# uga-ssrl/SSRLCV

Measured on AMD Instinct MI355X. Metric: Mpix/s SIFT extract (+ Mmatches/s 128-D brute-force, see `matcher`), higher is better.
Workload: dtype f32; 1 GPU; 2-view 4096x4096 pair per GPU (tools/scene.py pinhole views (PCG32 terrain + texture through Image::Camera)): SIFT_FeatureFactory::generateFeatures (sparse DoG path) on each image, pixels resident in HBM; images_per_gpu=2, parallelism=image-pair shard, library=release build (libssrlcv_hip_release.so)

## Files before the change

### ssrlcv_amd/csrc/keypoints.hip

```cpp
#include <hip/hip_runtime.h>
#include <float.h>
#include <math.h>
#include <stdlib.h>
#include "compact.h"
#include "dev_switch.h"
#include "scan_lookback.h"
#include "device_math.h"
#include "sift_plan.h"
#include "ssrlcv_hip.h"

using svp::OctaveState;

namespace {

struct LevelSet {
  const float* lvl[svp::kGauss];
  const float* lvlMinMax;
  const float* minmax;
  const float2* polar;
  int w, h;
};

struct DogView {
  const float* lo;
// ... 473 lines not shown
  }
  tab->total = pos;
}
__device__ __forceinline__ int range_of(const RangeTable* tab, uint32_t u) {
  int r = 0;
#pragma unroll
  for (int k = 1; k < 20; ++k)
    if (tab->start[k] <= u) r = k;
  return r;
}

struct OctaveSet {
  LevelSet L[svp::kOctaves];
  const ssrlcv_sskeypoint* kps[svp::kOctaves];
  float pixelWidth[svp::kOctaves];
  float* thetas[svp::kOctaves];
  uint32_t* thetaCnt[svp::kOctaves];
  const void* consts[svp::kOctaves];
};

template <int MAXO, int LPKS>
__global__ __launch_bounds__(64) void k_thetas(const OctaveState* states, const RangeTable* tab, OctaveSet set, float lambda,
                                               float orientationThreshold) {
  constexpr int LANES = 1 << LPKS, PER_BLOCK = 64 >> LPKS, CW = kThetaChunk * LANES;
  __shared__ float s_hist[36][PER_BLOCK];
  if (blockIdx.x >= tab->total) return;
  const int range = __builtin_amdgcn_readfirstlane(range_of(tab, blockIdx.x));
  const int octave = range & 3, useg = kSegOrder[range >> 2];
  const LevelSet& L = set.L[octave];
  const float pixelWidth = set.pixelWidth[octave];
  const int t = threadIdx.x, sub = t & (LANES - 1), col = t >> LPKS;
  const float fsub2 = (float)(2 * sub);
  const uint32_t local = (blockIdx.x - tab->start[range]) * PER_BLOCK + (uint32_t)(t >> LPKS);
  const bool have = local < tab->count[range];
  const int gi = (int)(tab->first[range] + local);
  const float pi = SSRLCV_PI_F;
  const float rad10 = pi / 18.0f;
  const float inv10 = 1.0f / rad10;
  ssrlcv_sskeypoint kp;
  kp.loc.x = kp.loc.y = 0.0f;
  kp.sigma = 1.0f;
  if (have) kp = set.kps[octave][gi];
  const float kx = kp.loc.x, ky = kp.loc.y;
  const float windowWidth = ceilf(kp.sigma * 3.0f * lambda / pixelWidth);
  const float minx = kx - windowWidth, miny = ky - windowWidth, maxx = kx + windowWidth, maxy = ky + windowWidth;
  const bool inside = have && useg >= 1 && useg <= 3 &&
                      !(minx < 0.0f || miny < 0.0f || maxx >= (unsigned)(L.w - 1) || maxy >= (unsigned)(L.h - 1));
#pragma unroll
  for (int i = 0; i < 36 * PER_BLOCK / 64; ++i) (&s_hist[0][0])[i * 64 + t] = 0.0f;
  const float weight = 2.0f * lambda * lambda * kp.sigma * kp.sigma;
  const float rweight = 1.0f / weight;
  const int W = L.w;
  const size_t levelStride = svp::polar_level_stride(L.w, L.h);
  {
    const float2* base = L.polar + (size_t)(useg - 1) * levelStride;
    const __amdgpu_buffer_rsrc_t rsrc = __builtin_amdgcn_make_buffer_rsrc((void*)base, 0, (int)(uint32_t)(levelStride * 8), 0x00020000);
    typedef unsigned u32x4 __attribute__((ext_vector_type(4)));
    typedef unsigned u32x2 __attribute__((ext_vector_type(2)));
    struct Cursor { float x, y, ty2; unsigned rowoff; bool act; };
    Cursor cf;
    cf.x = minx;
    cf.y = miny;
    cf.ty2 = (miny - ky) * (miny - ky);
    cf.rowoff = (unsigned)round_pos(miny) * (unsigned)W + 1u;
    cf.act = inside;
    auto advance = [&](Cursor& c) {
      float xn = c.x + (float)CW;
      if (__any(c.act && !(c.x >= (float)CW))) {
        float ch = c.x;
#pragma unroll 8
        for (int i = 0; i < CW; ++i) ch += 1.0f;
        xn = c.x >= (float)CW ? xn : ch;
      }
      if (c.act) {
        if (xn <= maxx) {
          c.x = xn;
        } else {
          c.x = minx;
          c.y += 1.0f;
          if (!(c.y <= maxy)) c.act = false;
          const float ty = c.y - ky;
          c.ty2 = ty * ty;
          c.rowoff = (unsigned)round_pos(c.y) * (unsigned)W + 1u;
        }
      }
    };
    typedef u32x4 Chunk[kThetaChunk / 2];
    auto fetch = [&](const Cursor& c, Chunk& into) {
      if (!c.act) return;
      const unsigned off = (c.rowoff + (unsigned)round_pos(c.x)) * 8u + 16u * (unsigned)sub;
#pragma unroll
      for (int j = 0; j < kThetaChunk / 4; ++j) into[j] = __builtin_amdgcn_raw_buffer_load_b128(rsrc, (int)(off + 16u * LANES * j), 0, 0);
    };
    auto fetch_upper = [&](const Cursor& c, Chunk& into) {
      if (!c.act) return;
      const unsigned off = (c.rowoff + (unsigned)round_pos(c.x)) * 8u + 16u * (unsigned)sub;
#pragma unroll
      for (int j = kThetaChunk / 4; j < kThetaChunk / 2; ++j) into[j] = __builtin_amdgcn_raw_buffer_load_b128(rsrc, (int)(off + 16u * LANES * j), 0, 0);
    };
    auto wants_upper = [&](const Cursor& c) { return __any(c.act && c.x + (float)(CW / 2 - 1) <= maxx); };
    Chunk qa, qb;
    Cursor ca, cb;
#pragma unroll
    for (int j = 0; j < kThetaChunk / 2; ++j) qa[j] = qb[j] = u32x4{0u, 0u, 0u, 0u};
    ca = cf;
    fetch(cf, qa);
    if (wants_upper(cf)) fetch_upper(cf, qa);
    advance(cf);
    cb = cf;
    auto step = [&](Chunk& cur, const Cursor& cc, Chunk& nxt, Cursor& cn) __attribute__((always_inline)) {
      cn = cf;
      fetch(cf, nxt);
      if (wants_upper(cf)) fetch_upper(cf, nxt);
      advance(cf);
      float xs[kThetaChunk];
      float xlast = cc.x + (float)(CW - 1);
#pragma unroll
      for (int i = 0; i < kThetaChunk; ++i) xs[i] = cc.x + (fsub2 + (float)(((i >> 1) << (1 + LPKS)) | (i & 1)));
      if (__any(cc.act && !(cc.x >= (float)CW))) {
        float ch = cc.x;
        float xc[kThetaChunk];
#pragma unroll
        for (int sIdx = 0; sIdx < CW; ++sIdx) {
          const int q = (sIdx >> 1) & (LANES - 1), i = ((sIdx >> (1 + LPKS)) << 1) | (sIdx & 1);
          if (LANES == 1 || q == 0) xc[i] = ch;
          else xc[i] = sub == q ? ch : xc[i];
          if (sIdx + 1 < CW) ch += 1.0f;
        }
        const bool direct = cc.x >= (float)CW;
#pragma unroll
        for (int i = 0; i < kThetaChunk; ++i) xs[i] = direct ? xs[i] : xc[i];
        xlast = direct ? xlast : ch;
      }
      const float cty2 = cc.ty2;
      const unsigned crow = cc.rowoff;
      const bool cact = cc.act;
      const bool aligned = cc.x >= 4.0f && round_pos(xlast) == round_pos(cc.x) + (CW - 1);
      if (__any(cact && !aligned)) {
        if (cact && !aligned) {
#pragma unroll
          for (int i = 0; i < kThetaChunk; ++i) {
            u32x2 e = u32x2{0u, 0u};
            if (xs[i] <= maxx) e = __builtin_amdgcn_raw_buffer_load_b64(rsrc, (int)((crow + (unsigned)round_pos(xs[i])) * 8u), 0, 0);
            cur[i >> 1][(i & 1) * 2] = e[0];
            cur[i >> 1][(i & 1) * 2 + 1] = e[1];
          }
        }
      }
      auto weigh = [&](float ang, float xi, float& wgt, int& bin) {
        const float angle = fmod_2pi_above(ang + (2.0f * pi), 2.0f * pi);
        bin = (int)floorf(sv::exact_div3(angle, rad10, inv10));
        const float tx = xi - kx;
        wgt = sv::expf_nonpos(sv::exact_div5(-((tx * tx) + cty2), weight, rweight));
      };
      const bool upperHalf = __any(cact && xs[kThetaChunk / 2] <= maxx);
      float wg[kThetaChunk], mg[kThetaChunk];
      float* slot[kThetaChunk];
      auto weigh_half = [&](auto hc) __attribute__((always_inline)) {
        constexpr int i0 = decltype(hc)::value * (kThetaChunk / 2);
#pragma unroll
        for (int i = i0; i < i0 + kThetaChunk / 2; ++i) {
          const unsigned um = cur[i >> 1][(i & 1) * 2], ua = cur[i >> 1][(i & 1) * 2 + 1];
          int bin;
          weigh(__builtin_bit_cast(float, ua), xs[i], wg[i], bin);
          const bool counts = cact && xs[i] <= maxx && (unsigned)bin < 36u;
          slot[i] = &s_hist[counts ? bin : 0][col];
          mg[i] = counts ? __builtin_bit_cast(float, um) : 0.0f;
        }
      };
      auto vote_half = [&](auto hc) __attribute__((always_inline)) {
        constexpr int j0 = decltype(hc)::value * (kThetaChunk / 4);
#pragma unroll
        for (int j = j0; j < j0 + kThetaChunk / 4; ++j) {
#pragma unroll
          for (int q = 0; q < LANES; ++q) {
            if (LANES == 1 || sub == q) {
              const float h0 = *slot[2 * j], h1 = *slot[2 * j + 1];
              const float n0 = fmaf(mg[2 * j], wg[2 * j], h0);
              const float n1 = fmaf(mg[2 * j + 1], wg[2 * j + 1], slot[2 * j + 1] == slot[2 * j] ? n0 : h1);
              *slot[2 * j] = n0;
              *slot[2 * j + 1] = n1;
            }
            if (LANES > 1) __builtin_amdgcn_wave_barrier();
          }
        }
      };
      weigh_half(std::integral_constant<int, 0>{});
      if (upperHalf) weigh_half(std::integral_constant<int, 1>{});
      vote_half(std::integral_constant<int, 0>{});
      if (upperHalf) vote_half(std::integral_constant<int, 1>{});
    };
    while (__any(ca.act)) {
      step(qa, ca, qb, cb);
      if (!__any(cb.act)) break;
      step(qb, cb, qa, ca);
    }
  }
  uint32_t cnt = 0;
  float outTheta[MAXO];
#pragma unroll
  for (int i = 0; i < MAXO; ++i) outTheta[i] = -FLT_MAX;
  if (inside && sub == 0) {
    float maxHist = 0.0f;
    for (int i = 0; i < 36; ++i) {
      const float h = s_hist[i][col];
      if (h > maxHist) maxHist = h;
    }
    maxHist *= orientationThreshold;
    float bestMag[MAXO], bestTh[MAXO];
#pragma unroll
    for (int i = 0; i < MAXO; ++i) { bestMag[i] = 0.0f; bestTh[i] = 0.0f; }
    float hprev = s_hist[35][col], hb = s_hist[0][col];
    for (int b = 0; b < 36; ++b) {
      const float hnext = s_hist[b == 35 ? 0 : b + 1][col];
      if (!(hb < maxHist || hb < hprev || hb < hnext || hb < bestMag[MAXO - 1])) {
        float tmag = hb;
        float tt = (hprev - hnext) / (hprev - (2.0f * hb) + hnext);
        tt *= (pi / 36.0f);
        tt += (b * rad10);
        tt = fmodf(tt + (2.0f * pi), 2.0f * pi);
#pragma unroll
        for (int i = 0; i < MAXO; ++i) {
          if (tmag > bestMag[i]) {
#pragma unroll
            for (int ii = i; ii < MAXO; ++ii) {
              float m2 = bestMag[ii], t2 = bestTh[ii];
              bestMag[ii] = tmag;
              bestTh[ii] = tt;
              tmag = m2;
              tt = t2;
            }
          }
        }
      }
      hprev = hb;
      hb = hnext;
    }
#pragma unroll
    for (int i = 0; i < MAXO; ++i) {
      if (bestMag[i] != 0.0f) { outTheta[i] = bestTh[i]; cnt = i + 1; }
    }
  }
  if (have && sub == 0) {
#pragma unroll
    for (int i = 0; i < MAXO; ++i) set.thetas[octave][(size_t)gi * svp::kMaxOrient + i] = outTheta[i];
    set.thetaCnt[octave][gi] = cnt;
  }
}

__device__ __forceinline__ float uniform_f(float v) {
  return __builtin_bit_cast(float, __builtin_amdgcn_readfirstlane(__builtin_bit_cast(int, v)));
}
struct DescConst {
  float c, s;
  float windowWidth;
  float invExpDen;
  float voteScale;
  float invBin;
  uint32_t magic;
  int32_t segment;
};
static_assert(sizeof(DescConst) == 32, "one s_load_dwordx8");
__global__ __launch_bounds__(256) void k_desc_consts(const RangeTable* tab, OctaveSet set, float lambda, const OctaveState* states,
                                                     const GroupCtl* regularCtl) {
  const uint32_t total = tab->total;
  const bool fromTable = regularCtl != nullptr && regularCtl->regular != 0u;
  for (uint32_t u = blockIdx.x * 256 + threadIdx.x; u < total; u += gridDim.x * 256) {
    const int range = range_of(tab, u);
    const int octave = range & 3;
    const int i = (int)(tab->first[range] + (u - tab->start[range]));
    const ssrlcv_sskeypoint* kps = set.kps[octave];
    const float pixelWidth = set.pixelWidth[octave];
    DescConst* __restrict__ out = (DescConst*)const_cast<void*>(set.consts[octave]);
    DescConst d;
    const float theta = kps[i].theta;
    d.c = sv_cosf(-theta);
    d.s = sv_sinf(-theta);
    d.windowWidth = ceilf(kps[i].sigma * lambda / pixelWidth);
    d.invExpDen = 1.0f / (2.0f * d.windowWidth * d.windowWidth);
    int boundExp;
    (void)frexpf(1.4143f * ((d.windowWidth + 2.0f) * (d.windowWidth + 2.0f)), &boundExp);
    d.voteScale = ldexpf(1.0f, 31 - boundExp);
    d.invBin = 1.0f / (d.windowWidth / 2.0f);
    const unsigned wi = (unsigned)(int)d.windowWidth;
    d.magic = wi > 1u ? 0xFFFFFFFFu / wi + 1u : 0u;
    d.segment = fromTable ? kSegOrder[range >> 2] : segment_of(states + octave, i);
    out[i] = d;
  }
}

__device__ __forceinline__ unsigned vote_u32(float v) {
  int r;
  asm("v_cvt_rpi_i32_f32 %0, %1" : "=v"(r) : "v"(v));
  return (unsigned)r;
}

#ifndef SSRLCV_DESC_COPIES
#define SSRLCV_DESC_COPIES 8
#endif
constexpr int kDescCopies = SSRLCV_DESC_COPIES;
#ifndef SSRLCV_DESC_VGPRS
#define SSRLCV_DESC_VGPRS 64
#endif
__global__ __launch_bounds__(256) __attribute__((amdgpu_waves_per_eu(4, 8), amdgpu_num_vgpr(SSRLCV_DESC_VGPRS), amdgpu_num_sgpr(102))) void k_descriptors(const RangeTable* tab, OctaveSet set, const uint32_t* featBase,
                                                     ssrlcv_sift_feature* __restrict__ features, uint32_t maxFeatures) {
  __shared__ unsigned s_bins[4][(1 + 128 + 2) * kDescCopies];
  __shared__ __attribute__((aligned(8))) uint8_t s_bytes[4][128];
  const int lane = threadIdx.x & 63, wave = __builtin_amdgcn_readfirstlane(threadIdx.x >> 6);
  unsigned* bins = s_bins[wave] + kDescCopies;
  const int copy = lane & (kDescCopies - 1);
  const float pi = SSRLCV_PI_F;
  const float rad45 = pi / 4.0f;
  const float inv45 = 1.0f / rad45;
  const uint32_t totalUnits = tab->total;
  for (uint32_t unit = blockIdx.x * 4 + wave; unit < totalUnits; unit += gridDim.x * 4) {
    const int range = range_of(tab, unit);
    const int octave = range & 3;
    const int gi = (int)(tab->first[range] + (unit - tab->start[range]));
    const LevelSet& L = set.L[octave];
    const float pixelWidth = set.pixelWidth[octave];
    const float2* __restrict__ polar = L.polar;
    const DescConst dc = reinterpret_cast<const DescConst*>(set.consts[octave])[gi];
    const ssrlcv_sskeypoint kp = set.kps[octave][gi];
    const int seg = dc.segment;
    const float kx = kp.loc.x, ky = kp.loc.y;
    const float theta = kp.theta;
    const float windowWidth = dc.windowWidth;
    const float binWidth = windowWidth / 2.0f;
    const float c = dc.c, s = dc.s;
    const float2* __restrict__ pl = polar + (size_t)(seg - 1) * svp::polar_level_stride(L.w, L.h) + 1;
#pragma unroll
    for (int i = 0; i < 2 * kDescCopies; ++i) bins[i * 64 + lane] = 0u;
    f32x2 rc[16];
    {
      const int ci = lane & 15;
      const float hx = ((float)(ci >> 2) * 0.5f - 0.75f) * windowWidth, hy = ((float)(ci & 3) * 0.5f - 0.75f) * windowWidth;
      const float rx = (hx * c) + (hy * s), ry = (-hx * s) + (hy * c);
#pragma unroll
      for (int cell = 0; cell < 16; ++cell) {
        if ((cell >> 2) == 0 || (cell & 3) == 0) continue;
        rc[cell].x = __builtin_bit_cast(float, __builtin_amdgcn_readlane(__builtin_bit_cast(int, rx), cell));
        rc[cell].y = __builtin_bit_cast(float, __builtin_amdgcn_readlane(__builtin_bit_cast(int, ry), cell));
      }
    }
    const float expDen = 2.0f * windowWidth * windowWidth, invExpDen = dc.invExpDen, invBin = dc.invBin;
    const float voteScale = dc.voteScale;
    const int Wi = (int)windowWidth;
    const unsigned centreIdx = (unsigned)(Wi * (Wi + 1));
    const unsigned magic = dc.magic;
    auto sample = [&](unsigned idx, float& cx, float& cy, bool& ok) {
      const unsigned yq = Wi == 1 ? idx : __umulhi(idx, magic);
      const unsigned xq = idx - yq * (unsigned)Wi + 1u;
      const bool centre = idx >= centreIdx;
      const float x = centre ? 0.0f : (float)(int)xq;
      const float y = centre ? 0.0f : (float)(int)yq;
      cx = (x * c) + (y * s);
      cy = (-x * s) + (y * c);
      ok = idx <= centreIdx && fmaxf(fabsf(cx), fabsf(cy)) <= windowWidth;
    };
    auto gather = [&](float px, float py) { return polar_px(pl, L.w, round_coord(px), round_coord(py)); };
    auto split = [&](float2 pg, bool live, float& w0, float& w1, unsigned*& pa, float& ang, bool& odd) {
      ang = fmod_2pi_above(pg.y - theta + (2.0f * pi), 2.0f * pi);
      const float t45 = ang * inv45;
      const float fk = floorf(t45);
      const float u = t45 - fk;
      odd = live && !(u > 1.0e-4f && u < 0.9999f);
      int k0 = (int)fk;
      const float a0 = fabsf(ang - (fk * rad45)), a1 = fabsf(ang - ((fk + 1.0f) * rad45));
      w0 = (live && !odd && (unsigned)k0 < 8u) ? 1.0f - sv::exact_div3(a0, rad45, inv45) : 0.0f;
      w1 = (live && !odd && (unsigned)(k0 + 1) < 8u) ? 1.0f - sv::exact_div3(a1, rad45, inv45) : 0.0f;
      k0 = k0 < -1 ? -1 : k0;
      pa = bins + k0 * kDescCopies + copy;
    };
    float ncx, ncy;
    bool nok;
    sample((unsigned)lane, ncx, ncy, nok);
    float2 npg[4] = {make_float2(0.0f, 0.0f), make_float2(0.0f, 0.0f), make_float2(0.0f, 0.0f), make_float2(0.0f, 0.0f)};
    auto gather4 = [&]() {
      npg[0] = gather(ncx + kx, ncy + ky);
      npg[1] = gather(kx - ncy, ncx + ky);
      npg[2] = gather(kx - ncx, ky - ncy);
      npg[3] = gather(ncy + kx, ky - ncx);
    };
    if (nok) gather4();
    for (unsigned base = 0; base <= centreIdx; base += 64) {
      const float cx = ncx, cy = ncy;
      const bool ok = nok;
      const float2 pg0 = npg[0], pg1 = npg[1], pg2 = npg[2], pg3 = npg[3];
      const bool turned = ok && base + (unsigned)lane < centreIdx;
      sample(base + 64 + (unsigned)lane, ncx, ncy, nok);
      if (nok) gather4();
      const float r2n = -((cx * cx) + (cy * cy));
      const float g = sv::expf_nonpos(sv::exact_div3(r2n, expDen, invExpDen)) * voteScale;
      float a0, a1, b0, b1, c0, c1, d0, d1, angA, angB, angC, angD;
      bool oddA, oddB, oddC, oddD;
      unsigned *pa, *pb, *pc, *pd;
      split(pg0, ok, a0, a1, pa, angA, oddA);
      split(pg1, turned, b0, b1, pb, angB, oddB);
      split(pg2, turned, c0, c1, pc, angC, oddC);
      split(pg3, turned, d0, d1, pd, angD, oddD);
      const float magA = pg0.x * g, magB = pg1.x * g, magC = pg2.x * g, magD = pg3.x * g;
      const float bwl = ok ? binWidth : -1.0f;
#pragma unroll
      for (int cell = 0; cell < 16; ++cell) {
        const int nx = cell >> 2, ny = cell & 3;
        if (nx == 0 || ny == 0) continue;
        const int cellB = (3 - ny) * 4 + nx, cellC = 15 - cell, cellD = ny * 4 + (3 - nx);
        const float tx = fabsf(rc[cell].x - cx), ty = fabsf(rc[cell].y - cy);
        if (fmaxf(tx, ty) <= bwl) {
          const float wxy = (1.0f - sv::exact_div3(tx, binWidth, invBin)) * (1.0f - sv::exact_div3(ty, binWidth, invBin));
          atomicAdd(pa + cell * 8 * kDescCopies, vote_u32((wxy * a0) * magA));
          atomicAdd(pa + cell * 8 * kDescCopies + kDescCopies, vote_u32((wxy * a1) * magA));
          atomicAdd(pb + cellB * 8 * kDescCopies, vote_u32((wxy * b0) * magB));
          atomicAdd(pb + cellB * 8 * kDescCopies + kDescCopies, vote_u32((wxy * b1) * magB));
          atomicAdd(pc + cellC * 8 * kDescCopies, vote_u32((wxy * c0) * magC));
          atomicAdd(pc + cellC * 8 * kDescCopies + kDescCopies, vote_u32((wxy * c1) * magC));
          atomicAdd(pd + cellD * 8 * kDescCopies, vote_u32((wxy * d0) * magD));
          atomicAdd(pd + cellD * 8 * kDescCopies + kDescCopies, vote_u32((wxy * d1) * magD));
        }
      }
      if (__ballot(oddA || oddB || oddC || oddD) != 0ull) {
#pragma unroll 1
        for (int m = 0; m < 4; ++m) {
          const bool odd = m == 0 ? oddA : m == 1 ? oddB : m == 2 ? oddC : oddD;
          if (!odd) continue;
          const float mcx = m == 0 ? cx : m == 1 ? -cy : m == 2 ? -cx : cy;
          const float mcy = m == 0 ? cy : m == 1 ? cx : m == 2 ? -cy : -cx;
          const float mang = m == 0 ? angA : m == 1 ? angB : m == 2 ? angC : angD;
          const float mmag = m == 0 ? magA : m == 1 ? magB : m == 2 ? magC : magD;
#pragma unroll 1
          for (int cell = 0; cell < 16; ++cell) {
            const int ci = lane & 15;
            (void)ci;
            const float hx0 = ((float)(cell >> 2) * 0.5f - 0.75f) * windowWidth, hy0 = ((float)(cell & 3) * 0.5f - 0.75f) * windowWidth;
            const float rx = (hx0 * c) + (hy0 * s), ry = (-hx0 * s) + (hy0 * c);
            float hx = fabsf(rx - mcx), hy = fabsf(ry - mcy);
            if (hx <= binWidth && hy <= binWidth) {
              hx = hx / binWidth;
              hy = hy / binWidth;
              for (int k = 0; k < 8; ++k) {
                float angle = fabsf(mang - ((float)k * rad45));
                if (angle < rad45) {
                  angle /= rad45;
                  const float temp = (1.0f - hx) * (1.0f - hy) * (1.0f - angle) * mmag;
                  atomicAdd(bins + (cell * 8 + k) * kDescCopies + copy, vote_u32(temp));
                }
              }
            }
          }
        }
      }
    }
    __builtin_amdgcn_wave_barrier();
    unsigned t0 = 0u, t1 = 0u;
#pragma unroll
    for (int cpy = 0; cpy < kDescCopies; ++cpy) {
      t0 += bins[lane * kDescCopies + cpy];
      t1 += bins[(lane + 64) * kDescCopies + cpy];
    }
    float v0 = (float)t0, v1 = (float)t1;
    float sq = sqrtf(sv::wave_sum((v0 * v0) + (v1 * v1)));
    v0 = v0 / sq;
    v1 = v1 / sq;
    if (v0 > 0.2f) v0 = 0.2f;
    if (v1 > 0.2f) v1 = 0.2f;
    sq = sqrtf(sv::wave_sum((v0 * v0) + (v1 * v1)));
    {
      int b0 = lane, b1 = lane + 64;
      int o0 = (((b0 >> 3) & 3) * 4 + (b0 >> 5)) * 8 + (b0 & 7);
      int o1 = (((b1 >> 3) & 3) * 4 + (b1 >> 5)) * 8 + (b1 & 7);
      s_bytes[wave][o0] = (uint8_t)roundf(255.0f * v0 / sq);
      s_bytes[wave][o1] = (uint8_t)roundf(255.0f * v1 / sq);
    }
    __builtin_amdgcn_wave_barrier();
    const uint32_t fi = featBase[octave] + (uint32_t)gi;
    if (fi < maxFeatures) {
      ssrlcv_sift_feature* f = features + fi;
      if (lane < 16) *reinterpret_cast<uint2*>(&f->values[lane * 8]) = *reinterpret_cast<const uint2*>(&s_bytes[wave][lane * 8]);
      if (lane == 16) {
        f->parent = -1;
        f->theta = kp.theta;
        f->sigma = kp.sigma;
        f->loc.x = kp.loc.x * pixelWidth;
        f->loc.y = kp.loc.y * pixelWidth;
      }
    }
    __builtin_amdgcn_wave_barrier();
  }
}

LevelSet make_levels(const ssrlcv_sift_plan* plan, char* ws, int o) {
  LevelSet L;
  const svp::OctavePlan& oc = plan->oct[o];
  for (int b = 0; b < svp::kGauss; ++b) L.lvl[b] = (const float*)(ws + plan->off_gauss[o][b]);
  L.lvlMinMax = (const float*)(ws + plan->off_minmax) + (size_t)o * 2 * (svp::kGauss + svp::kDog);
  L.minmax = L.lvlMinMax + 2 * svp::kGauss;
  L.polar = (const float2*)(ws + oc.off_polar);
  L.w = (int)oc.w;
  L.h = (int)oc.h;
  return L;
}

void launch_polar(const ssrlcv_sift_plan* plan, char* ws, hipStream_t st, int oFirst = 0, int oLast = svp::kOctaves - 1) {
  PolarJobs jobs;
  uint32_t pos = 0;
  for (int o = 0; o < svp::kOctaves; ++o) {
    const svp::OctavePlan& oc = plan->oct[o];
    jobs.L[o] = make_levels(plan, ws, o);
    jobs.out[o] = (float2*)(ws + oc.off_polar);
    jobs.start[o] = pos;
    jobs.tilesX[o] = (oc.w + 255) / 256;
    if (o >= oFirst && o <= oLast) pos += jobs.tilesX[o] * ((oc.h + kPolRows - 1) / kPolRows);
  }
  jobs.start[svp::kOctaves] = pos;
  hipLaunchKernelGGL(k_polar, dim3(pos), dim3(256), 0, st, jobs);
}

}
namespace svp {
void launch_polar_octave(const ssrlcv_sift_plan* plan, char* ws, int octave, hipStream_t st) {
  PolarJobs jobs;
  const svp::OctavePlan& oc = plan->oct[octave];
  const uint32_t tilesX = (oc.w + 255) / 256, tiles = tilesX * ((oc.h + kPolRows - 1) / kPolRows);
  for (int o = 0; o < svp::kOctaves; ++o) {
    jobs.L[o] = make_levels(plan, ws, octave);
    jobs.out[o] = (float2*)(ws + oc.off_polar);
    jobs.tilesX[o] = tilesX;
    jobs.start[o] = o <= octave ? 0u : tiles;
  }
  jobs.start[svp::kOctaves] = tiles;
  hipLaunchKernelGGL(k_polar, dim3(tiles), dim3(256), 0, st, jobs);
}
}
namespace {
hipError_t run_discard(OctaveState* st, const ssrlcv_sskeypoint* src, ssrlcv_sskeypoint* dst, uint32_t cap,
                       uint32_t* words, hipStream_t stream) {
  const OctaveState* cst = st;
  auto keyfn = [=] __device__(uint32_t i) -> uint32_t {
    if (!cst->hasExtrema || (int)i >= cst->n) return 0u;
    if (src[i].discard) return 0u;
    return 1u << segment_of(cst, (int)i);
  };
  auto emit = [=] __device__(uint32_t i, int, uint32_t d) { dst[d] = src[i]; };
  uint32_t* totals = nullptr;
  auto post = [=] __device__(const uint32_t* tot) { book_discard(st, tot); };
  return svc::partition<svp::kDog, 8>(cap, keyfn, emit, words, &totals, stream, &st->n, 1u, post);
}

constexpr unsigned kWaveKernelOversubscription = 16;
inline unsigned list_blocks(uint32_t cap) {
  unsigned b = (cap + 255) / 256;
  return b > 1024 ? 1024 : b;
}

}

extern "C" {

int ssrlcv_sift_plan_keypoints(const ssrlcv_sift_plan* plan, void* workspace, int octave, ssrlcv_sskeypoint** list,
                               int** blurIndices_dev) {
  if (!plan || !workspace || octave < 0 || octave >= svp::kOctaves) return SSRLCV_ERR_INVALID_ARG;
  char* ws = (char*)workspace;
  if (list) *list = (ssrlcv_sskeypoint*)(ws + (plan->listInB[octave] ? plan->oct[octave].off_kpB : plan->oct[octave].off_kpA));
  if (blurIndices_dev) *blurIndices_dev = (int*)(ws + plan->off_state + sizeof(OctaveState) * octave);
  return SSRLCV_OK;
}

int ssrlcv_sift_plan_overflow(const ssrlcv_sift_plan* plan, const void* workspace, uint32_t* octaveMask,
                              ssrlcv_stream_t stream) {
  if (!plan || !workspace || !octaveMask) return SSRLCV_ERR_INVALID_ARG;
  OctaveState st[svp::kOctaves];
  SSRLCV_HIP_TRY(hipMemcpyAsync(st, (const char*)workspace + plan->off_state, sizeof st, hipMemcpyDeviceToHost,
                                (hipStream_t)stream));
  SSRLCV_HIP_TRY(hipStreamSynchronize((hipStream_t)stream));
  uint32_t m = 0;
  for (int o = 0; o < svp::kOctaves; ++o)
    if (st[o].overflow) m |= 1u << o;
  *octaveMask = m;
  return m ? SSRLCV_ERR_CAPACITY : SSRLCV_OK;
}

}
namespace {

struct ListCtx {
  const ssrlcv_sift_plan* plan;
  const svp::OctavePlan* oc;
  int o;
  hipStream_t s;
  OctaveState* st;
  LevelSet L;
  ssrlcv_sskeypoint *A, *B;
  uint8_t* flags;
  uint32_t* words;
  uint32_t cap;
  ssrlcv_sskeypoint* cur() const { return plan->listInB[o] ? B : A; }
  ssrlcv_sskeypoint* oth() const { return plan->listInB[o] ? A : B; }
  void flip() const { plan->listInB[o] ^= 1; }
};
ListCtx make_ctx(const ssrlcv_sift_plan* plan, char* ws, int o, hipStream_t s) {
  ListCtx c;
  c.plan = plan;
  c.oc = &plan->oct[o];
  c.o = o;
  c.s = s;
  c.st = (OctaveState*)(ws + plan->off_state) + o;
  c.L = make_levels(plan, ws, o);
  c.A = (ssrlcv_sskeypoint*)(ws + c.oc->off_kpA);
  c.B = (ssrlcv_sskeypoint*)(ws + c.oc->off_kpB);
  c.flags = (uint8_t*)(ws + c.oc->off_flags);
  c.words = (uint32_t*)(ws + c.oc->off_part);
  c.cap = c.oc->cap;
  return c;
}

int stage_extrema(const ListCtx& c, bool afterFirstNoise) {
  hipLaunchKernelGGL(k_state_reset, dim3(1), dim3(1), 0, c.s, c.st);
  c.plan->listInB[c.o] = 0;
  const uint32_t P = c.oc->w * c.oc->h, cap = c.cap;
  const int W = (int)c.oc->w;
  const int octaveId = c.o;
  const float s1 = c.oc->sigma[1], s2 = c.oc->sigma[2], s3 = c.oc->sigma[3];
  const LevelSet Lc = c.L;
  ssrlcv_sskeypoint* first = c.A;
  auto emit = [=] __device__(uint32_t p, int b, uint32_t d) {
    if (d >= cap) return;
    ssrlcv_sskeypoint kp;
    kp.octave = octaveId;
    kp.blur = (int)b + 1;
    kp.loc.x = (float)(p % W);
    kp.loc.y = (float)(p / W);
    kp.intensity = dog_view(Lc, b + 1).raw(p);
    kp.sigma = b == 0 ? s1 : b == 1 ? s2 : s3;
    kp.theta = -1.0f;
    kp.discard = 0;
    first[d] = kp;
  };
  uint32_t* totals = nullptr;
  hipError_t e = svc::partition_flags<3>(P, c.flags, afterFirstNoise ? svp::kNoiseFlagShift : 0, emit, c.words, &totals, c.s);
  if (e != hipSuccess) return (int)e;
  hipLaunchKernelGGL(k_book_extrema, dim3(1), dim3(1), 0, c.s, c.st, totals, cap);
  return SSRLCV_OK;
}
int discard_flagged(const ListCtx& c) {
  hipError_t e = run_discard(c.st, c.cur(), c.oth(), c.cap, c.words, c.s);
  if (e != hipSuccess) return (int)e;
  c.flip();
  return SSRLCV_OK;
}
int stage_noise(const ListCtx& c, float threshold) {
  hipLaunchKernelGGL(k_flag_noise, dim3(list_blocks(c.cap)), dim3(256), 0, c.s, c.st, c.cur(), threshold);
  return discard_flagged(c);
}
int stage_refine(const ListCtx& c) {
  hipLaunchKernelGGL(k_refine, dim3(list_blocks(c.cap)), dim3(256), 0, c.s, c.st, c.cur(), c.L, c.oc->sigma[0],
                     c.oc->sigma[1] / c.oc->sigma[0]);
  int rc = discard_flagged(c);
  if (rc) return rc;
  OctaveState* st = c.st;
  const OctaveState* cst = c.st;
  const ssrlcv_sskeypoint* src = c.cur();
  ssrlcv_sskeypoint* dst = c.oth();
  auto keyfn = [=] __device__(uint32_t i) -> uint32_t {
    if (!cst->hasExtrema || (int)i >= cst->n) return 0u;
    int b = src[i].blur;
    return (b < 0 || b >= svp::kDog) ? 0u : (1u << b);
  };
  auto emit = [=] __device__(uint32_t i, int, uint32_t d) { dst[d] = src[i]; };
  uint32_t* totals = nullptr;
  auto post = [=] __device__(const uint32_t* tot) { book_rescan(st, tot); };
  hipError_t e = svc::partition<svp::kDog, 8>(c.cap, keyfn, emit, c.words, &totals, c.s, &st->n, 1u, post);
  if (e != hipSuccess) return (int)e;
  c.flip();
  return SSRLCV_OK;
}
int stage_edges(const ListCtx& c) {
  hipLaunchKernelGGL(k_flag_edges, dim3(list_blocks(c.cap)), dim3(256), 0, c.s, c.st, c.cur(), c.L, svp::kEdgeThreshold);
  return discard_flagged(c);
}
int stage_window(const ListCtx& c) {
  hipLaunchKernelGGL(k_flag_window, dim3(list_blocks(c.cap)), dim3(256), 0, c.s, c.st, c.cur(), c.L.w, c.L.h, c.oc->pixelWidth,
                     c.plan->params.descriptorContribWidth);
  return discard_flagged(c);
}
int stage_noise_edges_window(const ListCtx& c) {
  hipLaunchKernelGGL(k_flag_noise_edges_window, dim3(list_blocks(c.cap)), dim3(256), 0, c.s, c.st, c.cur(), c.L, svp::kNoiseThreshold,
                     svp::kEdgeThreshold, c.oc->pixelWidth, c.plan->params.descriptorContribWidth);
  return discard_flagged(c);
}

OctaveSet make_set(const ssrlcv_sift_plan* plan, char* ws) {
  OctaveSet set;
  for (int o = 0; o < svp::kOctaves; ++o) {
    const svp::OctavePlan& oc = plan->oct[o];
    set.L[o] = make_levels(plan, ws, o);
    set.kps[o] = (const ssrlcv_sskeypoint*)(ws + (plan->listInB[o] ? oc.off_kpB : oc.off_kpA));
    set.pixelWidth[o] = oc.pixelWidth;
    set.thetas[o] = (float*)(ws + oc.off_theta);
    set.thetaCnt[o] = (uint32_t*)(ws + oc.off_thetaCnt);
    set.consts[o] = ws + oc.off_descConst;
  }
  return set;
}

constexpr int kExpandItems = 16;
__global__ __launch_bounds__(svs::kThreads) void k_expand_orient(OctaveState* st, const ssrlcv_sskeypoint* __restrict__ src,
                                                                 ssrlcv_sskeypoint* __restrict__ dst, const float* __restrict__ thetas,
                                                                 const uint32_t* __restrict__ thetaCnt, uint32_t maxO, uint32_t cap,
                                                                 svs::TileScan<1> ts, GroupCtl* ctl, int g, int pieces) {
  constexpr int ITEMS = kExpandItems;
  constexpr uint32_t kTile = svs::kThreads * ITEMS;
  const uint32_t n = st->hasExtrema && st->n > 0 ? (uint32_t)st->n : 0u;
  uint32_t lo = 0, hi = n;
  if (pieces > 1) {
    if (g > 0) lo = ctl->cut[g - 1] < n ? ctl->cut[g - 1] : n;
    if (g + 1 < pieces) hi = ctl->cut[g] < n ? ctl->cut[g] : n;
    if (hi < lo) hi = lo;
  }
  const uint32_t e0 = lo * maxO, e1 = hi * maxO;
  const uint32_t tiles = (e1 - e0 + kTile - 1) / kTile;
  const uint32_t before = ctl->totals[g];
  uint32_t segFirst[svp::kDog];
// ... 856 lines not shown
```

Measured before the change: 3585 Mpix/s.

## Compact descriptor cell voting via LDS cell table and bitmask loop, halve VGPR cap

The unrolled 9-cell vote loop, which issued eight LDS atomics per cell under divergent branches, becomes two steps. First a bitmask of the cells that pass is built, then a ctz-driven loop reads each cell's rotated centre and precomputed byte offsets from a small per-wave LDS table. The VGPR limit for k_descriptors is halved to allow more waves per SIMD. This cuts code size, register pressure and divergent predicated atomics. The cost is an extra LDS read per cell and possible spills under the tighter register cap.

```diff
diff --git a/ssrlcv_amd/csrc/keypoints.hip b/ssrlcv_amd/csrc/keypoints.hip
--- a/ssrlcv_amd/csrc/keypoints.hip
+++ b/ssrlcv_amd/csrc/keypoints.hip
@@ -799,10 +799,12 @@
 #ifndef SSRLCV_DESC_VGPRS
 #define SSRLCV_DESC_VGPRS 64
 #endif
-__global__ __launch_bounds__(256) __attribute__((amdgpu_waves_per_eu(4, 8), amdgpu_num_vgpr(SSRLCV_DESC_VGPRS), amdgpu_num_sgpr(102))) void k_descriptors(const RangeTable* tab, OctaveSet set, const uint32_t* featBase,
+__global__ __launch_bounds__(256) __attribute__((amdgpu_waves_per_eu(4, 8), amdgpu_num_vgpr(SSRLCV_DESC_VGPRS / 2), amdgpu_num_sgpr(102))) void k_descriptors(const RangeTable* tab, OctaveSet set, const uint32_t* featBase,
                                                      ssrlcv_sift_feature* __restrict__ features, uint32_t maxFeatures) {
   __shared__ unsigned s_bins[4][(1 + 128 + 2) * kDescCopies];
   __shared__ __attribute__((aligned(8))) uint8_t s_bytes[4][128];
+  __shared__ uint4 s_cells[4][9];
+  constexpr int kCellBytes = 8 * kDescCopies * (int)sizeof(unsigned);
   const int lane = threadIdx.x & 63, wave = __builtin_amdgcn_readfirstlane(threadIdx.x >> 6);
   unsigned* bins = s_bins[wave] + kDescCopies;
   const int copy = lane & (kDescCopies - 1);
@@ -839,6 +841,12 @@
         rc[cell].x = __builtin_bit_cast(float, __builtin_amdgcn_readlane(__builtin_bit_cast(int, rx), cell));
         rc[cell].y = __builtin_bit_cast(float, __builtin_amdgcn_readlane(__builtin_bit_cast(int, ry), cell));
       }
+      const int nx = ci >> 2, ny = ci & 3;
+      if (lane < 16 && nx != 0 && ny != 0)
+        s_cells[wave][(nx - 1) * 3 + (ny - 1)] =
+            make_uint4(__builtin_bit_cast(unsigned, rx), __builtin_bit_cast(unsigned, ry),
+                       (unsigned)(ci * kCellBytes) | ((unsigned)(((3 - ny) * 4 + nx) * kCellBytes) << 16), 0u);
+      __builtin_amdgcn_wave_barrier();
     }
     const float expDen = 2.0f * windowWidth * windowWidth, invExpDen = dc.invExpDen, invBin = dc.invBin;
     const float voteScale = dc.voteScale;
@@ -898,23 +906,38 @@
       split(pg3, turned, d0, d1, pd, angD, oddD);
       const float magA = pg0.x * g, magB = pg1.x * g, magC = pg2.x * g, magD = pg3.x * g;
       const float bwl = ok ? binWidth : -1.0f;
+      unsigned todo = 0u;
 #pragma unroll
       for (int cell = 0; cell < 16; ++cell) {
         const int nx = cell >> 2, ny = cell & 3;
         if (nx == 0 || ny == 0) continue;
-        const int cellB = (3 - ny) * 4 + nx, cellC = 15 - cell, cellD = ny * 4 + (3 - nx);
         const float tx = fabsf(rc[cell].x - cx), ty = fabsf(rc[cell].y - cy);
-        if (fmaxf(tx, ty) <= bwl) {
-          const float wxy = (1.0f - sv::exact_div3(tx, binWidth, invBin)) * (1.0f - sv::exact_div3(ty, binWidth, invBin));
-          atomicAdd(pa + cell * 8 * kDescCopies, vote_u32((wxy * a0) * magA));
-          atomicAdd(pa + cell * 8 * kDescCopies + kDescCopies, vote_u32((wxy * a1) * magA));
-          atomicAdd(pb + cellB * 8 * kDescCopies, vote_u32((wxy * b0) * magB));
-          atomicAdd(pb + cellB * 8 * kDescCopies + kDescCopies, vote_u32((wxy * b1) * magB));
-          atomicAdd(pc + cellC * 8 * kDescCopies, vote_u32((wxy * c0) * magC));
-          atomicAdd(pc + cellC * 8 * kDescCopies + kDescCopies, vote_u32((wxy * c1) * magC));
-          atomicAdd(pd + cellD * 8 * kDescCopies, vote_u32((wxy * d0) * magD));
-          atomicAdd(pd + cellD * 8 * kDescCopies + kDescCopies, vote_u32((wxy * d1) * magD));
-        }
+        if (fmaxf(tx, ty) <= bwl) todo |= 1u << ((nx - 1) * 3 + (ny - 1));
+      }
+      unsigned* const pcEnd = pc + 15 * 8 * kDescCopies;
+      unsigned* const pdEnd = pd + 15 * 8 * kDescCopies;
+      while (todo != 0u) {
+        const uint4* const pe = &s_cells[wave][__builtin_ctz(todo)];
+        const uint3 e = make_uint3(pe->x, pe->y, pe->z);
+        todo &= todo - 1u;
+        const float tx = fabsf(__builtin_bit_cast(float, e.x) - cx), ty = fabsf(__builtin_bit_cast(float, e.y) - cy);
+        const float wxy = (1.0f - sv::exact_div3(tx, binWidth, invBin)) * (1.0f - sv::exact_div3(ty, binWidth, invBin));
+        const unsigned offA = e.z & 0xFFFFu, offB = e.z >> 16;
+        unsigned* const qa = (unsigned*)((char*)pa + offA);
+        unsigned* const qb = (unsigned*)((char*)pb + offB);
+        unsigned* const qc = (unsigned*)((char*)pcEnd - offA);
+        unsigned* const qd = (unsigned*)((char*)pdEnd - offB);
+        atomicAdd(qa, vote_u32((wxy * a0) * magA));
+        atomicAdd(qa + kDescCopies, vote_u32((wxy * a1) * magA));
+        __builtin_amdgcn_sched_barrier(0);
+        atomicAdd(qb, vote_u32((wxy * b0) * magB));
+        atomicAdd(qb + kDescCopies, vote_u32((wxy * b1) * magB));
+        __builtin_amdgcn_sched_barrier(0);
+        atomicAdd(qc, vote_u32((wxy * c0) * magC));
+        atomicAdd(qc + kDescCopies, vote_u32((wxy * c1) * magC));
+        __builtin_amdgcn_sched_barrier(0);
+        atomicAdd(qd, vote_u32((wxy * d0) * magD));
+        atomicAdd(qd + kDescCopies, vote_u32((wxy * d1) * magD));
       }
       if (__ballot(oddA || oddB || oddC || oddD) != 0ull) {
 #pragma unroll 1
```

New measurement: 3595 Mpix/s (median of 6 runs). Within noise of the previous version (+0.3%).
